# houzhijian/CONE

Measured on AMD Instinct MI355X. Metric: windows/sec + queries/sec, Ego4D-NLQ win_len=90 d=256 top-k=20, higher is better.
Workload: dtype f32

## Files before the change

cone_amd/_lib.py:

```python
from __future__ import annotations

import ctypes as C
import os

HERE = os.path.dirname(os.path.abspath(__file__))
LIB_PATH = os.path.join(HERE, "libcone_hip.so")

MAX_LAYERS = 8
MAX_PROJ = 3

c_float_p = C.c_void_p


class Linear(C.Structure):
    _fields_ = [("w", C.c_void_p), ("b", C.c_void_p)]


class LNorm(C.Structure):
    _fields_ = [("g", C.c_void_p), ("b", C.c_void_p)]


class Mha(C.Structure):
    _fields_ = [("in_proj_w", C.c_void_p), ("in_proj_b", C.c_void_p), ("out_proj", Linear)]

# ... 73 lines not shown
    "cone_topk_windows_workspace": (C.c_size_t, [C.c_int, C.c_int64, C.c_int]),
    "cone_topk_windows_ws": (C.c_int, [C.c_void_p, C.c_int, C.c_int64, C.c_int, C.c_void_p, C.c_void_p, C.c_void_p,
                                       C.c_size_t, C.c_void_p]),
    "cone_project_workspace": (C.c_size_t, [C.c_void_p, C.c_int, C.c_int64]),
    "cone_project_tokens": (C.c_int, [C.c_void_p, C.c_int, C.c_void_p, C.c_int64, C.c_void_p, C.c_void_p,
                                      C.c_size_t, C.c_void_p]),
    "cone_mask_lengths": (C.c_int, [C.c_void_p, C.c_int, C.c_int, C.c_void_p, C.c_void_p]),
    "cone_forward_workspace": (C.c_size_t, [C.c_void_p, C.c_int, C.c_int, C.c_int]),
    "cone_forward_windows": (C.c_int, [C.c_void_p, C.c_void_p, C.c_void_p, C.c_void_p, C.c_void_p, C.c_int,
                                       C.c_int, C.c_int, C.c_void_p, C.c_void_p, C.c_void_p, C.POINTER(Taps),
                                       C.c_void_p, C.c_size_t, C.c_void_p]),
    "cone_forward_packed_workspace": (C.c_size_t, [C.c_void_p, C.c_int, C.c_int, C.c_int, C.POINTER(Layer0)]),
    "cone_forward_packed": (C.c_int, [C.c_void_p, C.c_void_p, C.c_void_p, C.c_void_p, C.c_void_p, C.c_void_p,
                                      C.c_void_p, C.c_int, C.c_int, C.c_int, C.c_void_p, C.c_void_p, C.c_void_p,
                                      C.POINTER(Taps), C.POINTER(Layer0), C.c_void_p, C.c_size_t, C.c_void_p]),
    "cone_pos_table_rows": (C.c_int64, [C.c_int]),
    "cone_pos_tables": (C.c_int, [C.c_void_p, C.c_int, C.c_void_p, C.c_void_p, C.c_void_p]),
    "cone_layer0_project_workspace": (C.c_size_t, [C.c_void_p, C.c_int64]),
    "cone_layer0_project": (C.c_int, [C.c_void_p, C.c_void_p, C.c_int64, C.c_void_p, C.c_void_p, C.c_size_t, C.c_void_p]),
    "cone_layer0_text_positions": (C.c_int, [C.c_void_p, C.c_void_p, C.c_void_p, C.c_int64, C.c_void_p, C.c_void_p, C.c_void_p]),
    "cone_clip_matching_workspace": (C.c_size_t, [C.c_void_p, C.c_int]),
    "cone_clip_matching_gathered": (C.c_int, [C.c_void_p, C.c_void_p, C.c_void_p, C.c_void_p, C.c_void_p,
                                              C.c_void_p, C.c_void_p, C.c_void_p, C.c_int, C.c_void_p,
                                              C.c_void_p, C.c_size_t, C.c_void_p]),
    "cone_clip_matching": (C.c_int, [C.c_void_p, C.c_void_p, C.c_void_p, C.c_void_p, C.c_int, C.c_void_p,
                                     C.c_int, C.c_void_p, C.c_void_p, C.c_size_t, C.c_void_p]),
    "cone_window_table": (C.c_int, [C.c_void_p, C.c_int, C.c_int, C.c_void_p, C.c_void_p, C.c_int] + [C.c_void_p] * 4 + [C.c_int] * 3
                          + [C.c_void_p, C.c_int, C.c_int] + [C.c_void_p] * 7 + [C.c_void_p]),
    "cone_compose_rows": (C.c_int, [C.c_void_p, C.c_void_p, C.c_void_p, C.c_void_p, C.c_void_p, C.c_float,
                                    C.c_int, C.c_int, C.c_int, C.c_void_p, C.c_void_p]),
    "cone_fuse_nms": (C.c_int, [C.c_void_p, C.c_void_p, C.c_void_p, C.c_int, C.c_int, C.c_double, C.c_int, C.c_int,
                                C.c_void_p, C.c_void_p, C.c_void_p, C.c_void_p]),
    "cone_fuse_nms_f64": (C.c_int, [C.c_void_p, C.c_void_p, C.c_void_p, C.c_int, C.c_int, C.c_double, C.c_int, C.c_int,
                                    C.c_void_p, C.c_void_p, C.c_void_p, C.c_void_p]),
    "cone_temporal_nms": (C.c_int, [C.c_void_p, C.c_int, C.c_double, C.c_int, C.c_void_p, C.c_void_p,
                                    C.c_void_p]),
    "cone_matcher_cost": (C.c_int, [C.c_void_p, C.c_void_p, C.c_void_p, C.c_int, C.c_int, C.c_float, C.c_float,
                                    C.c_float, C.c_void_p, C.c_void_p, C.c_void_p]),
    "cone_criterion_forward": (C.c_int, [C.c_void_p, C.c_void_p, C.c_void_p, C.c_void_p, C.c_void_p, C.c_void_p, C.c_int,
                                         C.c_void_p, C.c_void_p, C.c_int, C.c_void_p, C.c_int, C.c_int, C.c_int,
                                         C.c_float, C.c_float, C.c_float, C.c_float, C.c_float, C.c_void_p, C.c_void_p,
                                         C.c_void_p, C.c_void_p]),
    "cone_adapter_nce": (C.c_int, [C.c_void_p, C.c_int, C.c_float, C.c_void_p, C.c_void_p]),
    "cone_prof_enable": (C.c_int, [C.c_int]),
    "cone_prof_collect": (C.c_int64, [C.c_void_p, C.c_int64]),
    "cone_eval_recall": (C.c_int, [C.c_void_p, C.c_void_p, C.c_void_p, C.c_int, C.c_int, C.c_void_p, C.c_int,
                                   C.c_void_p, C.c_int, C.c_int, C.c_void_p, C.c_void_p, C.c_void_p]),
    "cone_eval_window_recall": (C.c_int, [C.c_void_p, C.c_int, C.c_int, C.c_void_p, C.c_double, C.c_int, C.c_void_p,
                                          C.c_int, C.c_void_p, C.c_void_p]),
    "cone_model_set_option": (C.c_int, [C.c_void_p, C.c_char_p, C.c_int]),
    "cone_test_gemm": (C.c_int, [C.c_void_p, C.c_void_p, C.c_int, C.c_void_p, C.c_void_p, C.c_void_p,
                                 C.c_void_p, C.c_void_p, C.c_void_p, C.c_void_p, C.c_void_p, C.c_int, C.c_int,
                                 C.c_int, C.c_int, C.c_void_p]),
    "cone_test_gemm_bf16_image_bytes": (C.c_size_t, [C.c_int, C.c_int]),
    "cone_test_gemm_bf16": (C.c_int, [C.c_void_p, C.c_void_p, C.c_int, C.c_void_p, C.c_void_p, C.c_void_p,
                                      C.c_void_p, C.c_void_p, C.c_void_p, C.c_void_p, C.c_void_p, C.c_int, C.c_int,
                                      C.c_int, C.c_int, C.c_void_p, C.c_int, C.c_int, C.c_void_p, C.c_void_p]),
    "cone_test_ffn": (C.c_int, [C.c_void_p] * 8 + [C.c_int, C.c_int, C.c_void_p]),
    "cone_test_proj_ffn": (C.c_int, [C.c_void_p] * 13 + [C.c_int, C.c_int, C.c_void_p]),
    "cone_test_tail_form": (C.c_int, [C.c_void_p] * 13 + [C.c_int, C.c_int] + [C.c_void_p] * 3 + [C.c_int, C.c_void_p, C.c_int, C.c_int,
                                                                               C.c_void_p, C.c_void_p]),
    "cone_test_proj_ffn_spread_scratch_bytes": (C.c_size_t, [C.c_int]),
    "cone_test_proj_ffn_spread": (C.c_int, [C.c_void_p] * 13 + [C.c_int, C.c_int, C.c_void_p, C.c_void_p]),
    "cone_test_ffn_split_image_bytes": (C.c_size_t, [C.c_int]),
    "cone_test_ffn_split": (C.c_int, [C.c_void_p] * 8 + [C.c_int, C.c_int, C.c_void_p, C.c_int, C.c_void_p]),
    "cone_test_rows_split_image_bytes": (C.c_size_t, [C.c_int]),
    "cone_test_rows_split": (C.c_int, [C.c_void_p] * 4 + [C.c_int, C.c_int, C.c_void_p, C.c_int, C.c_void_p]),
    "cone_test_proj_split_image_bytes": (C.c_size_t, []),
    "cone_test_proj_ffn_split": (C.c_int, [C.c_void_p] * 13 + [C.c_int, C.c_int, C.c_void_p, C.c_void_p, C.c_int, C.c_void_p]),
    "cone_test_enc_attn": (C.c_int, [C.c_int] + [C.c_void_p] * 9 + [C.c_int, C.c_int, C.c_int, C.c_void_p]),
    "cone_test_dec_cross": (C.c_int, [C.c_void_p] * 9 + [C.c_int] * 4 + [C.c_void_p, C.c_void_p]),
    "cone_test_dec_cross_slab_floats": (C.c_size_t, []),
    "cone_test_enc_attn_txt": (C.c_int, [C.c_int] + [C.c_void_p] * 10 + [C.c_int, C.c_int, C.c_int, C.c_void_p]),
    "cone_test_small_attn": (C.c_int, [C.c_void_p, C.c_int, C.c_void_p, C.c_int, C.c_void_p, C.c_int, C.c_void_p, C.c_int,
                                       C.c_void_p, C.c_int, C.c_int, C.c_int, C.c_void_p]),
    "cone_test_dec_cross_ex": (C.c_int, [C.c_void_p] * 10 + [C.c_int] * 4 + [C.c_void_p] * 4 + [C.c_int, C.c_void_p]),
    "cone_test_layernorm": (C.c_int, [C.c_void_p, C.c_void_p, C.c_void_p, C.c_void_p, C.c_int64, C.c_int,
                                      C.c_void_p]),
    "cone_test_gen_attn": (C.c_int, [C.c_void_p, C.c_int, C.c_void_p, C.c_int, C.c_void_p, C.c_int, C.c_void_p, C.c_int,
                                     C.c_void_p, C.c_void_p] + [C.c_int] * 5 + [C.c_void_p]),
    "cone_test_grid_limit_y": (C.c_int, []),
    "cone_test_scan_lengths": (C.c_int, [C.c_void_p, C.c_void_p, C.c_int, C.c_void_p, C.c_void_p]),
    "cone_test_compact_index": (C.c_int, [C.c_void_p, C.c_void_p, C.c_int, C.c_void_p, C.c_void_p, C.c_void_p, C.c_int,
                                          C.c_void_p, C.c_int, C.c_void_p]),
    "cone_test_pack_pos": (C.c_int, [C.c_void_p] * 11 + [C.c_int, C.c_int] + [C.c_void_p] * 4),
    "cone_test_gen_pack_pos": (C.c_int, [C.c_void_p] * 10 + [C.c_int] * 3 + [C.c_void_p] * 4),
    "cone_test_pack_l0": (C.c_int, [C.c_void_p] * 15 + [C.c_int, C.c_int, C.c_void_p]),
    "cone_test_row_index": (C.c_int, [C.c_void_p] * 6 + [C.c_int, C.c_int, C.c_void_p]),
    "cone_test_add_pos_rows": (C.c_int, [C.c_void_p] * 5 + [C.c_int, C.c_int] + [C.c_void_p] * 3),
    "cone_test_txt_pos_rows": (C.c_int, [C.c_void_p] * 3 + [C.c_int, C.c_int] + [C.c_void_p] * 3 + [C.c_int] + [C.c_void_p] * 3),
    "cone_test_gen_txt_pos_rows": (C.c_int, [C.c_void_p] * 3 + [C.c_int, C.c_int] + [C.c_void_p] * 3 + [C.c_int, C.c_void_p, C.c_int,
                                                                                                    C.c_void_p, C.c_void_p]),
    "cone_test_saliency": (C.c_int, [C.c_void_p] * 7 + [C.c_int, C.c_void_p, C.c_int, C.c_int, C.c_void_p]),
    "cone_test_gen_saliency": (C.c_int, [C.c_void_p] * 7 + [C.c_int, C.c_void_p, C.c_int, C.c_int, C.c_int, C.c_void_p]),
    "cone_test_rowdot": (C.c_int, [C.c_void_p, C.c_int, C.c_void_p, C.c_void_p, C.c_void_p, C.c_int, C.c_int64, C.c_int, C.c_int,
                                   C.c_void_p]),
    "cone_test_gen_rowdot": (C.c_int, [C.c_void_p, C.c_int, C.c_void_p, C.c_void_p, C.c_void_p, C.c_int, C.c_int64, C.c_int, C.c_int,
                                       C.c_int, C.c_void_p]),
    "cone_test_tile_rows": (C.c_int, [C.c_void_p, C.c_int, C.c_int64, C.c_void_p]),
    "cone_test_tile_rows2": (C.c_int, [C.c_void_p] * 4 + [C.c_int, C.c_int64, C.c_void_p]),
}
EXPORTS = tuple(_SIGNATURES)

_lib = None


# ... 66 lines not shown
```

cone_amd/build.py:

```python
from __future__ import annotations

import os
import subprocess
import sys
from concurrent.futures import ThreadPoolExecutor

HERE = os.path.dirname(os.path.abspath(__file__))
CSRC = os.path.join(HERE, "csrc")
OBJ = os.path.join(CSRC, "_obj")
LIB = os.path.join(HERE, "libcone_hip.so")
PYLISTS = os.path.join(HERE, "_cone_pylists.so")
SOURCES = ["api.hip", "gemm.hip", "rowops.hip", "attention.hip", "window_ops.hip", "prefilter.hip",
           "postproc.hip", "prof.hip", "dec_cross.hip", "metrics.hip", "ffn.hip", "criterion.hip", "dec_cross_mfma.hip", "ffn_split.hip", "ffn_wide.hip",
           "general.hip", "ffn_bf16.hip", "gemm_bf16.hip"]
FLAGS = ["-O3", "--offload-arch=gfx950", "-fPIC", "-std=c++17", "-Wall", "-Wno-unused-function"]
NO_CONTRACT = {"window_ops.hip", "postproc.hip", "metrics.hip", "criterion.hip", "general.hip"}


def _deps_mtime():
    hdrs = [os.path.join(CSRC, f) for f in os.listdir(CSRC) if f.endswith(".h")]
    hdrs += [os.path.join(HERE, "..", "include", "cone_hip.h"), __file__]
    return max(os.path.getmtime(h) for h in hdrs)


def _compile(src):
    obj = os.path.join(OBJ, src.replace(".hip", ".o"))
    stamp = obj + ".flags"
    path = os.path.join(CSRC, src)
    extra = ["-ffp-contract=off"] if src in NO_CONTRACT else []
    extra += os.environ.get("CONE_HIPCC_FLAGS", "").split()
    flags = " ".join([*FLAGS, *extra])
    try:
        with open(stamp) as f:
            same_flags = f.read() == flags
    except OSError:
        same_flags = False
    if same_flags and os.path.exists(obj) and os.path.getmtime(obj) >= max(os.path.getmtime(path), _deps_mtime()):
        return obj
    cmd = ["hipcc", *FLAGS, *extra, "-c", path, "-o", obj]
    r = subprocess.run(cmd, capture_output=True, text=True)
    if r.returncode != 0:
        raise RuntimeError(f"hipcc failed for {src}:\n{r.stdout}\n{r.stderr}")
    with open(stamp, "w") as f:
        f.write(flags)
    if r.stderr.strip():
        sys.stderr.write(r.stderr)
    return obj


def build(force: bool = False) -> str:
    os.makedirs(OBJ, exist_ok=True)
    if force:
        for f in os.listdir(OBJ):
            os.remove(os.path.join(OBJ, f))
    with ThreadPoolExecutor(max_workers=4) as ex:
        objs = list(ex.map(_compile, SOURCES))
    if (not os.path.exists(LIB)) or any(os.path.getmtime(o) > os.path.getmtime(LIB) for o in objs):
        r = subprocess.run(["hipcc", "--offload-arch=gfx950", "-shared", "-fPIC", "-o", LIB, *objs],
                           capture_output=True, text=True)
        if r.returncode != 0:
            raise RuntimeError(f"link failed:\n{r.stdout}\n{r.stderr}")
    try:
        build_pylists()
    except (RuntimeError, OSError) as e:
        try:
            if os.path.exists(PYLISTS) and os.path.getmtime(PYLISTS) < os.path.getmtime(os.path.join(CSRC, "pylists.c")):
                os.remove(PYLISTS)
# ... 22 lines not shown
```

cone_amd/csrc/api.hip:

```cpp
#include <stdarg.h>
#include <string.h>

#include <vector>

#include "common.h"
#include "rows_chain.h"

namespace cone {

static thread_local char g_err[512] = "";
void set_error(const char* fmt, ...) {
    va_list ap;
    va_start(ap, fmt);
    vsnprintf(g_err, sizeof(g_err), fmt, ap);
    va_end(ap);
}

struct Linear { const float* w = nullptr; const float* b = nullptr; };
struct LNorm { const float* g = nullptr; const float* b = nullptr; };
struct Mha { const float* in_w = nullptr; const float* in_b = nullptr; Linear out; };
struct EncLayer { Mha sa; Linear l1, l2; LNorm n1, n2; };
struct DecLayer { Mha sa, ca; Linear l1, l2; LNorm n1, n2, n3; };

}

struct cone_model {
    int d, heads, ff, n_enc, n_dec, nq, n_proj, dt, dv, dvm, has_adapter;
    float* arena = nullptr;
    cone::LNorm vproj_ln[CONE_MAX_PROJ], tproj_ln[CONE_MAX_PROJ];
    cone::Linear vproj[CONE_MAX_PROJ], tproj[CONE_MAX_PROJ];
    cone::EncLayer enc[CONE_MAX_LAYERS];
    cone::DecLayer dec[CONE_MAX_LAYERS];
    cone::LNorm dec_norm;
    const float* query_embed = nullptr;
    cone::Linear class_embed, span[3], saliency, adapter[2];
    const float* dim_t = nullptr;
    const float* txt_pos_emb = nullptr; int txt_pos_rows = 0; cone::LNorm txt_pos_ln;
    int pre_norm = 0; cone::LNorm enc_norm;
    cone::Linear dec_k, dec_v;
    const float* dec_vT[CONE_MAX_LAYERS] = {};
    float* dec0_tgt1 = nullptr; float* dec0_dq = nullptr; float* dec0_scratch = nullptr;
    float* dec_sa_tab[CONE_MAX_LAYERS] = {}; float* dec_ca_tab[CONE_MAX_LAYERS] = {};
    float* tab_arena = nullptr; const float* tab_pos_rows = nullptr; const float* tab_pos_qk = nullptr; int tab_max_v_l = 0;
    int opt_dec_fold = 2;
    int opt_dec0_const = 1;
    int opt_l0_gather = 1;
    int opt_pos_tables = 1;
    int opt_gemm = 0;
    cone::TailWeights enc_tail[CONE_MAX_LAYERS] = {}, dec_tail[CONE_MAX_LAYERS] = {};
    char* split_img = nullptr; char* bf16_img = nullptr;
    int opt_qkv_fused = 1;
    int opt_split_bf16 = 0;
    int opt_bf16 = 0;
    int opt_res_gather = 1;
    int opt_spread = 1;
    int opt_chain = 1;
    int opt_ffn_fused = 2;
    int gen_native = 0;
// ... 1528 lines not shown
                                      void* stream) {
    return launch_gen_pack_pos(vproj, vrow0, vlen, tproj, trow0, qlen, off, dim_t, X, POS, d, B, Lmax, (hipStream_t)stream, tpe,
                               tpg, tpb);
}
extern "C" int cone_test_pack_l0(const float* vproj, const int32_t* vrow0, const int32_t* vlen, const float* tproj,
                                 const int32_t* trow0, const int32_t* qlen, const int32_t* off, const float* dim_t,
                                 const float* qkv_vid, const float* qkv_txt, const float* pos_qk, float* X, float* POS, float* QK,
                                 float* V, int B, int Lmax, void* stream) {
    return launch_pack_l0(vproj, vrow0, vlen, tproj, trow0, qlen, off, dim_t, qkv_vid, qkv_txt, pos_qk, X, POS, QK, V, B, Lmax,
                          (hipStream_t)stream);
}
extern "C" int cone_test_row_index(const int32_t* vrow0, const int32_t* vlen, const int32_t* trow0, const int32_t* qlen,
                                   const int32_t* off, int32_t* ridx, int B, int Lmax, void* stream) {
    return launch_row_index(vrow0, vlen, trow0, qlen, off, ridx, B, Lmax, (hipStream_t)stream);
}
extern "C" int cone_test_add_pos_rows(const float* MEM, const int32_t* off, const int32_t* vlen, const float* pos_rows, float* XP,
                                      int B, int Lmax, const float* txt_pos, const int32_t* trow0, void* stream) {
    return launch_add_pos_rows(MEM, off, vlen, pos_rows, XP, B, Lmax, (hipStream_t)stream, txt_pos, trow0);
}
extern "C" int cone_test_txt_pos_rows(const float* tproj, const int32_t* tok_index, const int32_t* src_row, int mod, int n_emb,
                                      const float* tpe, const float* tpg, const float* tpb, int n, const int32_t* n_dev,
                                      float* out, void* stream) {
    return launch_txt_pos_rows(tproj, tok_index, src_row, mod, n_emb, tpe, tpg, tpb, n, n_dev, out, (hipStream_t)stream);
}
extern "C" int cone_test_gen_txt_pos_rows(const float* tproj, const int32_t* tok_index, const int32_t* src_row, int mod, int n_emb,
                                          const float* tpe, const float* tpg, const float* tpb, int n, const int32_t* n_dev, int d,
                                          float* out, void* stream) {
    return launch_gen_txt_pos_rows(tproj, tok_index, src_row, mod, n_emb, tpe, tpg, tpb, n, n_dev, d, out, (hipStream_t)stream);
}
extern "C" int cone_test_saliency(const float* MEM, const int32_t* off, const int32_t* vlen, const int32_t* qlen, const float* w,
                                  const float* bias, float* sal, int Lv_out, float* mem_tap, int Lq_out, int B, void* stream) {
    return launch_saliency(MEM, off, vlen, qlen, w, bias, sal, Lv_out, mem_tap, Lq_out, B, (hipStream_t)stream);
}
extern "C" int cone_test_gen_saliency(const float* MEM, const int32_t* off, const int32_t* vlen, const int32_t* qlen,
                                      const float* w, const float* bias, float* sal, int Lv_out, float* mem_tap, int Lq_out, int B,
                                      int d, void* stream) {
    return launch_gen_saliency(MEM, off, vlen, qlen, w, bias, sal, Lv_out, mem_tap, Lq_out, B, d, (hipStream_t)stream);
}
extern "C" int cone_test_rowdot(const float* X, int ldx, const float* W, const float* b, float* out, int ldo, int64_t n_rows,
                                int nout, int act, void* stream) {
    return launch_rowdot(X, ldx, W, b, out, ldo, n_rows, nout, act, (hipStream_t)stream);
}
extern "C" int cone_test_gen_rowdot(const float* X, int ldx, const float* W, const float* b, float* out, int ldo, int64_t n_rows,
                                    int nout, int act, int d, void* stream) {
    return launch_gen_rowdot(X, ldx, W, b, out, ldo, n_rows, nout, act, d, (hipStream_t)stream);
}
extern "C" int cone_test_tile_rows(float* x, int period, int64_t n_rows, void* stream) {
    return launch_tile_rows(x, period, n_rows, (hipStream_t)stream);
}
extern "C" int cone_test_tile_rows2(float* d0, const float* s0, float* d1, const float* s1, int period, int64_t n_rows,
                                    void* stream) {
    return launch_tile_rows2(d0, s0, d1, s1, period, n_rows, (hipStream_t)stream);
}
```

cone_amd/csrc/gemm.hip:

```cpp
#include <mutex>

#include "common.h"
#include "rows_chain.h"

#ifndef CONE_GEMM_NT_STORE
#define CONE_GEMM_NT_STORE 0
#endif

namespace cone {

constexpr int BK = 32;

template <int BM, int BN, bool HAS_A2>
__global__ __launch_bounds__(256, 2) void gemm_f32_kernel(GemmArgs p) {
    constexpr int WAVES_N = BN / 64;
    constexpr int LDA_S = BM + 1, LDB_S = BN + 1;
    constexpr int A_PASSES = BM / 32, B_PASSES = BN / 32;
    __shared__ float smem[BK * LDA_S + BK * LDB_S];
    float* As = smem;
    float* Bs = smem + BK * LDA_S;

    int M = p.M;
    if (p.M_dev) { int md = *p.M_dev; M = md < M ? md : M; }
    const int m0 = blockIdx.x * BM;
    if (m0 >= M) return;
    const int n0 = blockIdx.y * BN;
    const int N = p.N, K = p.K;

    const int tid = threadIdx.x;
    const int lane = tid & 63;
    const int wave = tid >> 6;
    const int wm = wave / WAVES_N, wn = wave % WAVES_N;
    const int li = lane & 31, lh = lane >> 5;

    const int lrow = tid >> 3;
    const int lkc = tid & 7;

    float4 ra[A_PASSES], rb[B_PASSES];

    auto gload = [&](int kt) {
        const int kof = kt * BK + lkc * 4;
#pragma unroll
        for (int ps = 0; ps < A_PASSES; ++ps) {
            int row = m0 + lrow + 32 * ps;
            row = row < M ? row : M - 1;
            float4 v = *reinterpret_cast<const float4*>(p.A + (size_t)row * p.lda + kof);
            if (HAS_A2) {
                const int r2 = p.a2_mod ? row % p.a2_mod : row;
                const float4 w = *reinterpret_cast<const float4*>(p.A2 + (size_t)r2 * p.lda2 + kof);
                v.x += w.x; v.y += w.y; v.z += w.z; v.w += w.w;
            }
            ra[ps] = v;
        }
#pragma unroll
        for (int ps = 0; ps < B_PASSES; ++ps) {
// ... 293 lines not shown
#pragma unroll
    for (int g = 0; g < 4; ++g) {
        __builtin_amdgcn_wave_barrier();
#pragma unroll
        for (int t = 0; t < 8; ++t)
#pragma unroll
            for (int rr4 = 0; rr4 < 4; ++rr4)
                ep[(rr4 + 4 * lh) * RT_EP_LD + t * 32 + li] = acc[t][4 * g + rr4];
        __builtin_amdgcn_wave_barrier();
        float4 v[8], rr[8], ad[8];
#pragma unroll
        for (int k = 0; k < 8; ++k) {
            int i = min(8 * g + k, rows_here - 1);
            i = i < 0 ? 0 : i;
            const size_t m = (size_t)min(mrow0 + i, M - 1);
            if (flags & EPI_RESIDUAL) rr[k] = *reinterpret_cast<const float4*>(p.R + (p.r_mod ? m % (size_t)p.r_mod : m) * p.ldr + n0 + c4);
            if (p.C2) ad[k] = *reinterpret_cast<const float4*>(p.ADD + m * p.ldc + n0 + c4);
            v[k] = *reinterpret_cast<const float4*>(ep + k * RT_EP_LD + c4);
        }
#pragma unroll
        for (int k = 0; k < 8; ++k) {
            float4 x = v[k];
            x.x += bias4.x; x.y += bias4.y; x.z += bias4.z; x.w += bias4.w;
            if (flags & EPI_RELU) { x.x = fmaxf(x.x, 0.f); x.y = fmaxf(x.y, 0.f); x.z = fmaxf(x.z, 0.f); x.w = fmaxf(x.w, 0.f); }
            if (flags & EPI_RESIDUAL) { x.x += rr[k].x; x.y += rr[k].y; x.z += rr[k].z; x.w += rr[k].w; }
            if (flags & EPI_LN) {
                const float mean = wave_sum_dpp((x.x + x.y) + (x.z + x.w)) * (1.0f / 256.0f);
                const float d0 = x.x - mean, d1 = x.y - mean, d2 = x.z - mean, d3 = x.w - mean;
                const float var = wave_sum_dpp((d0 * d0 + d1 * d1) + (d2 * d2 + d3 * d3)) * (1.0f / 256.0f);
                const float rstd = 1.0f / sqrtf(var + 1e-5f);
                x.x = d0 * rstd * g4.x + be4.x; x.y = d1 * rstd * g4.y + be4.y;
                x.z = d2 * rstd * g4.z + be4.z; x.w = d3 * rstd * g4.w + be4.w;
            }
            if (8 * g + k < rows_here) {
                const size_t m = (size_t)(mrow0 + 8 * g + k);
                *reinterpret_cast<float4*>(p.C + m * p.ldc + n0 + c4) = x;
                if (p.C2) {
                    x.x += ad[k].x; x.y += ad[k].y; x.z += ad[k].z; x.w += ad[k].w;
                    *reinterpret_cast<float4*>(p.C2 + m * p.ldc + n0 + c4) = x;
                }
            }
        }
    }
}

typedef float f32x4a __attribute__((ext_vector_type(4)));

__device__ __forceinline__ int swz16(int row) { return (0x1230 >> (((row >> 2) & 3) * 4)) & 3; }

__global__ __launch_bounds__(512, 4) void gemm_rows16_kernel(GemmArgs p) {
    constexpr int RBK = 16, SLAB = (RT_BM + RT_BN) * RBK, NBUF = 3, NPIECE = 3;
    extern __shared__ __attribute__((aligned(16))) float smem[];
    int M = p.M;
    if (p.M_dev) { int md = *p.M_dev; M = md < M ? md : M; }
    const int nc = p.N / RT_BN;
    const int L = blockIdx.x, grp = L / (8 * nc), r0 = L % (8 * nc);
    const int m0 = (grp * 8 + (r0 & 7)) * RT_BM;
    if (m0 >= M) return;
    const int n0 = (r0 >> 3) * RT_BN;
    const int K = p.K;
    const int tid = threadIdx.x, lane = tid & 63;
    const int wave = __builtin_amdgcn_readfirstlane(tid >> 6);
    const int li = lane & 15, lg = lane >> 4;

    const float* __restrict__ Ab = p.A + (size_t)m0 * p.lda;
    const float* __restrict__ Wb = p.W + (size_t)n0 * p.ldw;
    const float* src[NPIECE];
    int dst[NPIECE];
#pragma unroll
    for (int i = 0; i < NPIECE; ++i) {
        const int q = wave * NPIECE + i;
        const int row = q * 16 + lane / 4;
        const int chunk = (lane % 4) ^ swz16(row);
        if (q < 8) {
            const int sr = (m0 + row < M) ? row : (M - 1 - m0);
            src[i] = Ab + (size_t)sr * p.lda + (chunk << 2);
        } else {
            src[i] = Wb + (size_t)(row - RT_BM) * p.ldw + (chunk << 2);
        }
        dst[i] = q * 256;
    }
    auto stream_piece = [&](int kt, int buf, int i) { GLDS16(src[i] + kt * RBK, smem + buf * SLAB + dst[i]); };

    f32x4a acc[16];
#pragma unroll
    for (int t = 0; t < 16; ++t) acc[t] = f32x4a{0.f, 0.f, 0.f, 0.f};
    const int csw = (lg ^ swz16(li)) << 2;
    const int a_row = (wave * 16 + li) * RBK + csw;
    const int b_row = RT_BM * RBK + li * RBK + csw;

    const int nk = K / RBK;
#pragma unroll
    for (int i = 0; i < NPIECE; ++i) stream_piece(0, 0, i);
    if (nk > 1) {
#pragma unroll
        for (int i = 0; i < NPIECE; ++i) stream_piece(1, 1, i);
        asm volatile("s_waitcnt vmcnt(%0)" ::"n"(NPIECE) : "memory");
    } else {
        asm volatile("s_waitcnt vmcnt(0)" ::: "memory");
    }
    __builtin_amdgcn_s_barrier();
    for (int kt = 0; kt < nk; ++kt) {
        const float* sb = smem + (kt % NBUF) * SLAB;
        const int nxt = (kt + 2) % NBUF;
        const bool more = kt + 2 < nk;
        const f32x4a a = *reinterpret_cast<const f32x4a*>(sb + a_row);
#pragma unroll
// ... 375 lines not shown
#pragma unroll
            for (int t = 0; t < 2; ++t)
#pragma unroll
                for (int r = 0; r < 4; ++r) ep[(4 * lg + r) * RS_EP_LD + 32 * wave + 16 * t + li] = acc[t][r];
            __syncthreads();
            const int flags = st.flags;
            float4 bias4 = make_float4(0.f, 0.f, 0.f, 0.f);
            if (st.bias) bias4 = *reinterpret_cast<const float4*>(st.bias + c4);
            float4 v[2], rr[2];
#pragma unroll
            for (int k = 0; k < 2; ++k) {
                const size_t m = (size_t)min(m0 + 2 * wave + k, M - 1);
                if (flags & EPI_RESIDUAL) rr[k] = *reinterpret_cast<const float4*>(st.R + m * st.ldr + c4);
                v[k] = *reinterpret_cast<const float4*>(ep + (2 * wave + k) * RS_EP_LD + c4);
            }
#pragma unroll
            for (int k = 0; k < 2; ++k) {
                float4 xx = v[k];
                xx.x += bias4.x; xx.y += bias4.y; xx.z += bias4.z; xx.w += bias4.w;
                if (flags & EPI_RELU) { xx.x = fmaxf(xx.x, 0.f); xx.y = fmaxf(xx.y, 0.f); xx.z = fmaxf(xx.z, 0.f); xx.w = fmaxf(xx.w, 0.f); }
                if (flags & EPI_RESIDUAL) { xx.x += rr[k].x; xx.y += rr[k].y; xx.z += rr[k].z; xx.w += rr[k].w; }
                x[k] = xx;
            }
        }
        in_regs = true;
#pragma unroll
        for (int k = 0; k < 2; ++k) {
            const int m = m0 + 2 * wave + k;
            if (st.C && m < M) *reinterpret_cast<float4*>(st.C + (size_t)m * st.ldc + c4) = x[k];
            if (st.hout) {
                for (int n = 0; n < st.hnout; ++n) {
                    const float4 xv = x[k];
                    const float4 wv = reinterpret_cast<const float4*>(st.hw + n * 256)[lane];
                    float s = __builtin_fmaf(xv.x, wv.x, xv.y * wv.y) + __builtin_fmaf(xv.z, wv.z, xv.w * wv.w);
                    s = wave_sum(s) + st.hb[n];
                    if (st.hact == 1) s = 1.0f / (1.0f + expf(-s));
                    if (lane == 0 && m < M) st.hout[(size_t)m * st.hld + n] = s;
                }
            }
        }
    }
    asm volatile("s_waitcnt vmcnt(0)" ::: "memory");
}


#ifndef CONE_RS_MAX_WGS
#define CONE_RS_MAX_WGS 1280
#endif
constexpr int RS_MAX_WGS = CONE_RS_MAX_WGS;
#ifndef CONE_RS_SPLIT_WGS
#define CONE_RS_SPLIT_WGS 256
#endif

int launch_gemm(const GemmArgs& a, hipStream_t s) {
    CONE_REQUIRE(a.K > 0 && a.K % BK == 0, "gemm: K=%d must be a multiple of %d", a.K, BK);
    CONE_REQUIRE(a.lda % 4 == 0 && a.ldw % 4 == 0, "gemm: lda/ldw must be multiples of 4");
    CONE_REQUIRE(!(a.flags & EPI_RESIDUAL) || a.R, "gemm: residual flag without R");
    if (a.M <= 0) return 0;
    if (a.flags & EPI_LN) CONE_REQUIRE(a.N == 256 && a.ln_g && a.ln_b, "gemm: LayerNorm epilogue needs N == 256");
    const bool rows_ok = a.N % 256 == 0 && !a.A2;
    const bool use_rows = rows_ok && a.variant != GEMM_SQUARE;
    const bool need_rows = a.C2 != nullptr;
    CONE_REQUIRE(!need_rows || (rows_ok && a.ADD), "gemm: second output needs the row tile (N %% 256 == 0, no A2)");
    if (use_rows || need_rows) {
        static DeviceOnce once;
        CONE_CHECK_HIP(device_once(once, [] {
            hipError_t rc = hipFuncSetAttribute((const void*)gemm_rows16_kernel, hipFuncAttributeMaxDynamicSharedMemorySize,
                                                RowTile<16>::LDS_BYTES);
            if (rc == hipSuccess)
                rc = hipFuncSetAttribute((const void*)gemm_rows_kernel<16>, hipFuncAttributeMaxDynamicSharedMemorySize,
                                         RowTile<16>::LDS_BYTES);
            if (rc == hipSuccess)
                rc = hipFuncSetAttribute((const void*)gemm_rows_small_kernel, hipFuncAttributeMaxDynamicSharedMemorySize, 160 * 1024);
            return rc;
        }));
        int n_cu = 0;
        CONE_CHECK_HIP(device_once(once, [] { return hipSuccess; }, &n_cu));
        const bool waves8 = a.variant != GEMM_ROWS4;
        const bool small_ok = waves8 && !a.C2 && a.variant == GEMM_AUTO && rs_lds_bytes(a.K) <= 160 * 1024;
        if (small_ok && (int64_t)((a.M + 15) / 16) * (a.N / RT_BN) > RS_MAX_WGS && a.m_off == 0) {
            const int nc = a.N / RT_BN;
            const int64_t G = (int64_t)((a.M + RT_BM - 1) / RT_BM) * nc;
            const int64_t m1 = G / n_cu * n_cu / nc * RT_BM;
            const int64_t rem = a.M - m1;
            if (m1 > 0 && rem > 0 && (rem + 15) / 16 * nc <= CONE_RS_SPLIT_WGS) {
                GemmArgs h = a;
                h.M = (int)m1;
                h.variant = GEMM_ROWS8;
                if (int rc = launch_gemm(h, s)) return rc;
                GemmArgs t = a;
                t.A = a.A + (size_t)m1 * a.lda; t.C = a.C + (size_t)m1 * a.ldc; t.M = (int)rem; t.m_off = (int)m1;
                if (a.R && !a.r_mod) t.R = a.R + (size_t)m1 * a.ldr;
                return launch_gemm(t, s);
            }
        }
        if (small_ok && !(a.flags & EPI_LN) && a.K <= 1024 && (a.M + 15) / 16 <= RSP_MAX_GROUPS &&
            (a.M + 15) / 16 * (a.N / 16) <= RSP_MAX_TILES && !(a.flags & GEMM_NO_SPREAD)) {
            ProfScope ps(PK_GEMM_ROWS_SMALL, a.M, a.N, a.K, a.M_dev, s, a.m_off);
            hipLaunchKernelGGL(gemm_rows_spread_kernel, dim3((unsigned)(a.N / 16), (unsigned)((a.M + 15) / 16)), dim3(64), 0, s, a);
            CONE_LAUNCH_CHECK();
            return 0;
        }
        if (small_ok && (int64_t)((a.M + 15) / 16) * (a.N / RT_BN) <= RS_MAX_WGS) {
            ProfScope ps(PK_GEMM_ROWS_SMALL, a.M, a.N, a.K, a.M_dev, s, a.m_off);
            hipLaunchKernelGGL(gemm_rows_small_kernel, dim3((unsigned)((a.M + 15) / 16), (unsigned)(a.N / RT_BN)), dim3(512),
                               rs_lds_bytes(a.K), s, a);
            CONE_LAUNCH_CHECK();
            return 0;
        }
        const int row_tiles = (a.M + RT_BM - 1) / RT_BM;
        dim3 grid((unsigned)((row_tiles + 7) / 8 * 8 * (a.N / RT_BN)));
        ProfScope ps(waves8 ? PK_GEMM_ROWS16 : PK_GEMM_ROWS, a.M, a.N, a.K, a.M_dev, s);
        if (waves8)
            hipLaunchKernelGGL(gemm_rows16_kernel, grid, dim3(512), RowTile<16>::LDS_BYTES, s, a);
        else
            hipLaunchKernelGGL(gemm_rows_kernel<16>, grid, dim3(256), RowTile<16>::LDS_BYTES, s, a);
        CONE_LAUNCH_CHECK();
        return 0;
    }
    if (a.flags & EPI_LN) {
        CONE_REQUIRE(a.N == 256 && a.ln_g && a.ln_b, "gemm: LayerNorm epilogue needs N == 256");
        CONE_REQUIRE(!a.A2, "gemm: LayerNorm epilogue with A2 is not instantiated");
        dim3 grid((a.M + 63) / 64, 1);
        ProfScope ps(PK_GEMM_64x256, a.M, a.N, a.K, a.M_dev, s);
        hipLaunchKernelGGL((gemm_f32_kernel<64, 256, false>), grid, dim3(256), 0, s, a);
    } else {
        dim3 grid((a.M + 127) / 128, (a.N + 127) / 128);
        ProfScope ps(a.A2 ? PK_GEMM_128x128_A2 : PK_GEMM_128x128, a.M, a.N, a.K, a.M_dev, s);
        if (a.A2) {
            CONE_REQUIRE(a.lda2 % 4 == 0, "gemm: lda2 must be a multiple of 4");
            hipLaunchKernelGGL((gemm_f32_kernel<128, 128, true>), grid, dim3(256), 0, s, a);
        } else {
            hipLaunchKernelGGL((gemm_f32_kernel<128, 128, false>), grid, dim3(256), 0, s, a);
        }
    }
    CONE_LAUNCH_CHECK();
    return 0;
}

bool rows_chain_supported(int M) { return M > 0 && (M + 15) / 16 <= RS_MAX_WGS; }
bool gemm_rows_spread_rows(int M) { return M > 0 && (M + 15) / 16 <= RSP_MAX_GROUPS; }

int launch_rows_chain(const ChainArgs& a, hipStream_t s) {
    CONE_REQUIRE(a.A && a.n_stages >= 1 && a.n_stages <= CHAIN_MAX_STAGES && a.lda % 4 == 0, "rows chain: bad arguments");
    if (a.M <= 0) return 0;
    CONE_REQUIRE(rows_chain_supported(a.M), "rows chain: %d rows are beyond the small-M regime", a.M);
    for (int i = 0; i < a.n_stages; ++i) {
        const ChainStage& st = a.st[i];
        if (st.kind == 0) {
            CONE_REQUIRE(st.W && st.K % 16 == 0 && st.K >= 16 && st.K <= 1024 && (i == 0 || st.K == 256),
                         "rows chain: stage %d: K=%d (stage 0: a multiple of 16 up to 1024; later stages: 256)", i, st.K);
            CONE_REQUIRE(!(st.flags & EPI_RESIDUAL) || (st.R && st.ldr % 4 == 0), "rows chain: residual flag without R");
            CONE_REQUIRE(!(st.flags & EPI_LN), "rows chain: a LayerNorm epilogue is a stage of its own (kind 1)");
        } else {
            CONE_REQUIRE(st.kind == 1 && st.ln_g && st.ln_b, "rows chain: stage %d: bad LayerNorm stage", i);
        }
        CONE_REQUIRE(!st.C || st.ldc % 4 == 0, "rows chain: output row stride must be a multiple of 4");
        CONE_REQUIRE(!st.hout || (st.hw && st.hb && st.hnout >= 1 && st.hnout <= 2), "rows chain: bad head");
    }
    CONE_REQUIRE(a.st[0].kind == 0 || a.lda >= 256, "rows chain: a LayerNorm first stage reads 256-wide rows");
    const int K0 = a.st[0].kind == 0 ? a.st[0].K : 256;
    const size_t lds = (size_t)((16 * K0 > 16 * RS_EP_LD ? 16 * K0 : 16 * RS_EP_LD) + 16 * RS_EP_LD + 8 * RS_RING) * sizeof(float);
    static DeviceOnce once;
    CONE_CHECK_HIP(device_once(once, [] {
        return hipFuncSetAttribute((const void*)rows_chain_kernel, hipFuncAttributeMaxDynamicSharedMemorySize, 160 * 1024);
    }));
    hipLaunchKernelGGL(rows_chain_kernel, dim3((unsigned)((a.M + 15) / 16)), dim3(512), lds, s, a);
    CONE_LAUNCH_CHECK();
    return 0;
}

}
```

include/cone_hip.h:

```cpp
#ifndef CONE_HIP_H
#define CONE_HIP_H

#include <stddef.h>
#include <stdint.h>

#ifdef __cplusplus
extern "C" {
#endif

#define CONE_HIP_ABI_VERSION 8

#define CONE_E_INVALID (-1)
#define CONE_E_HIP (-2)
#define CONE_E_WORKSPACE (-3)

#define CONE_MAX_LAYERS 8
#define CONE_MAX_PROJ 3
#define CONE_TABLE_MAX_V_L 255
#define CONE_MAX_WINDOW_TOKENS 256
#define CONE_MAX_LONG_WINDOW_TOKENS 1024

typedef struct cone_model cone_model;

typedef struct { const float* w; const float* b; } cone_linear_w;
// ... 133 lines not shown
                        const int32_t* txt_len, int B, int Lv_max, int Lq_max,
                        float* logits, float* spans, float* saliency, const cone_taps* taps,
                        const cone_layer0* l0 , void* ws, size_t ws_bytes, void* stream);

size_t cone_clip_matching_workspace(const cone_model* m, int B);
int cone_clip_matching_gathered(const cone_model* m, const float* cls, const int32_t* cls_row,
                                const float* vid, const int32_t* vid_row0, const int32_t* vid_len,
                                const int32_t* pad_len, const float* spans, int B, float* match,
                                void* ws, size_t ws_bytes, void* stream);
int cone_clip_matching(const cone_model* m, const float* cls, const float* vid, const int32_t* vid_len,
                       int Lv_pad, const float* spans, int B, float* match,
                       void* ws, size_t ws_bytes, void* stream);

int cone_compose_rows(const float* logits, const float* spans, const float* match,
                      const int32_t* duration, const int32_t* video_start, float clip_length,
                      int sort, int B, int Nq, float* rows, void* stream);


int cone_fuse_nms(const float* cand, const int64_t* cand_off, const int32_t* n_valid, int nq, int n_max,
                  double nms_thd, int max_before, int max_after, double* out_rows, int32_t* out_n, int32_t* out_idx,
                  void* stream);

int cone_fuse_nms_f64(const double* cand, const int64_t* cand_off, const int32_t* n_valid, int nq, int n_max,
                      double nms_thd, int max_before, int max_after, double* out_rows, int32_t* out_n, int32_t* out_idx,
                      void* stream);

int cone_temporal_nms(const double* pred, int n, double nms_thd, int max_after,
                      int32_t* keep_idx, int32_t* keep_n, void* stream);

int cone_matcher_cost(const float* logits, const float* spans, const float* tgt, int B, int Nq,
                      float cost_span, float cost_giou, float cost_class, float* cost, int32_t* best,
                      void* stream);

int cone_criterion_forward(const float* logits, const float* spans, const float* tgt, const int32_t* tgt_off,
                           const float* neg_logits, const float* saliency, int L, const int32_t* pos_idx,
                           const int32_t* neg_idx, int P, const float* neg_saliency, int L2, int B, int Nq,
                           float cost_span, float cost_giou, float cost_class, float eos_coef, float saliency_margin,
                           int32_t* assign, float* part, float* losses, void* stream);
int cone_adapter_nce(const float* sim, int n, float temperature, float* loss, void* stream);

int cone_eval_recall(const double* rows, const int32_t* n, const double* gt, int nq, int max_after,
                     const double* thresholds, int n_thr, const int32_t* topk, int n_topk, int mode,
                     int64_t* hits, double* top1_iou, void* stream);
int cone_eval_window_recall(const int32_t* win_idx, int nq, int k, const double* gt, double clip_length,
                            int slide, const int32_t* topk, int n_topk, int64_t* hits, void* stream);

int cone_prof_enable(int on);
int64_t cone_prof_collect(double* out, int64_t max_rec);

int cone_model_set_option(cone_model* m, const char* name, int value);
int cone_test_gemm(const float* A, const float* A2, int a2_mod, const float* W, const float* bias,
                   const float* R, const float* ln_g, const float* ln_b, float* C, float* C2,
                   const float* ADD, int M, int N, int K, int flags, void* stream);
size_t cone_test_gemm_bf16_image_bytes(int N, int K);
int cone_test_gemm_bf16(const float* A, const float* A2, int a2_mod, const float* W, const float* bias,
                        const float* R, const float* ln_g, const float* ln_b, float* C, float* C2,
                        const float* ADD, int M, int N, int K, int flags, void* img, int ldc, int r_mod,
                        const int32_t* M_dev, void* stream);
int cone_test_ffn(const float* X, const float* W1, const float* b1, const float* W2, const float* b2,
                  const float* ln_g, const float* ln_b, float* OUT, int M, int ff, void* stream);
int cone_test_proj_ffn(const float* A, const float* Wo, const float* bo, const float* R, const float* pg, const float* pb,
                       const float* W1, const float* b1, const float* W2, const float* b2, const float* ln_g,
                       const float* ln_b, float* OUT, int M, int ff, void* stream);
#define CONE_TEST_PACK 1
#define CONE_TEST_SINGLE_PIECE 2
size_t cone_test_ffn_split_image_bytes(int ff);
int cone_test_ffn_split(const float* X, const float* W1, const float* b1, const float* W2, const float* b2,
                        const float* ln_g, const float* ln_b, float* OUT, int M, int ff, void* img, int pack, void* stream);
size_t cone_test_rows_split_image_bytes(int N);
int cone_test_rows_split(const float* X, const float* W, const float* bias, float* C, int M, int N, void* img, int pack,
                         void* stream);
#define CONE_FFN_SPREAD_MAX_ROWS 1024
size_t cone_test_proj_ffn_spread_scratch_bytes(int ff);
int cone_test_proj_ffn_spread(const float* A, const float* Wo, const float* bo, const float* R, const float* pg, const float* pb,
                              const float* W1, const float* b1, const float* W2, const float* b2, const float* ln_g,
                              const float* ln_b, float* OUT, int M, int ff, void* scratch, void* stream);
enum { CONE_TAIL_FORM_ROWS128 = 0, CONE_TAIL_FORM_ROWS64 = 1, CONE_TAIL_FORM_WIDE = 2, CONE_TAIL_FORM_LADDER = 3,
       CONE_TAIL_FORM_SPREAD = 4 };
int cone_test_tail_form(const float* A, const float* Wo, const float* bo, const float* R, const float* pg, const float* pb,
                        const float* W1, const float* b1, const float* W2, const float* b2, const float* ln_g,
                        const float* ln_b, float* OUT, int M, int ff, const int32_t* r_idx, const float* R2,
                        const int32_t* M_dev, int pre, float* OUT2, int form, int n_cu, void* scratch, void* stream);
size_t cone_test_proj_split_image_bytes(void);
int cone_test_proj_ffn_split(const float* A, const float* Wo, const float* bo, const float* R, const float* pg,
                             const float* pb, const float* W1, const float* b1, const float* W2, const float* b2,
                             const float* ln_g, const float* ln_b, float* OUT, int M, int ff, void* img, void* wo_img,
                             int pack, void* stream);
int cone_test_enc_attn(int mode, const float* QKV, const float* qkv_vid, const float* qkv_txt, const float* pos_qk,
                       const int32_t* vrow0, const int32_t* vlen, const int32_t* trow0, const int32_t* off, float* OUT,
                       int B, int Lmax, int pos_zero_row , void* stream);
int cone_test_dec_cross(const float* DQ, const float* X, const float* pos_rows, const int32_t* vlen, const int32_t* off,
                        const float* Wk, const float* WvT, const float* bv, float* OUT, int B, int nq, int Lmax,
                        int variant, float* qk_slabs, void* stream);
size_t cone_test_dec_cross_slab_floats(void);
int cone_test_enc_attn_txt(int mode, const float* QKV, const float* qkv_vid, const float* qkv_txt, const float* pos_qk,
                           const float* txt_pos_qk, const int32_t* vrow0, const int32_t* vlen, const int32_t* trow0,
                           const int32_t* off, float* OUT, int B, int Lmax, int pos_zero_row, void* stream);
int cone_test_small_attn(const float* Q, int ldq, const float* K, int ldk, const float* V, int ldv, float* OUT, int ldo,
                         const int32_t* off, int B, int nq, int Lmax, void* stream);
int cone_test_dec_cross_ex(const float* DQ, const float* XP, const float* X, const float* pos_rows, const int32_t* vlen,
                           const int32_t* off, const float* Wk, const float* WvT, const float* bv, float* OUT, int B, int nq,
                           int Lmax, int variant, float* qk_slabs, const float* sal_w, const float* sal_b, float* sal,
                           int sal_ld, void* stream);
int cone_test_layernorm(const float* x, const float* g, const float* b, float* out, int64_t n_rows,
                        int dim, void* stream);
int cone_test_gen_attn(const float* Q, int ldq, const float* K, int ldk, const float* V, int ldv, float* OUT, int ldo,
// ... 41 lines not shown
```

Measured before the change: 376,200.

## Add persistent MFMA GEMM for K=256 bias-only projections with tail fallback

Result: no change. 379,100, median of 6 (+0.8%).

```diff
diff --git a/cone_amd/_lib.py b/cone_amd/_lib.py
--- a/cone_amd/_lib.py
+++ b/cone_amd/_lib.py
@@ -149,6 +149,9 @@
     "cone_test_gemm": (C.c_int, [C.c_void_p, C.c_void_p, C.c_int, C.c_void_p, C.c_void_p, C.c_void_p,
                                  C.c_void_p, C.c_void_p, C.c_void_p, C.c_void_p, C.c_void_p, C.c_int, C.c_int,
                                  C.c_int, C.c_int, C.c_void_p]),
+    "cone_test_gemm_ladder": (C.c_int, [C.c_void_p, C.c_void_p, C.c_int, C.c_void_p, C.c_void_p, C.c_void_p,
+                                        C.c_void_p, C.c_void_p, C.c_void_p, C.c_void_p, C.c_void_p, C.c_int, C.c_int,
+                                        C.c_int, C.c_int, C.c_int, C.c_void_p, C.c_int, C.c_void_p]),
     "cone_test_gemm_bf16_image_bytes": (C.c_size_t, [C.c_int, C.c_int]),
     "cone_test_gemm_bf16": (C.c_int, [C.c_void_p, C.c_void_p, C.c_int, C.c_void_p, C.c_void_p, C.c_void_p,
                                       C.c_void_p, C.c_void_p, C.c_void_p, C.c_void_p, C.c_void_p, C.c_int, C.c_int,
diff --git a/cone_amd/build.py b/cone_amd/build.py
--- a/cone_amd/build.py
+++ b/cone_amd/build.py
@@ -12,7 +12,7 @@
 PYLISTS = os.path.join(HERE, "_cone_pylists.so")
 SOURCES = ["api.hip", "gemm.hip", "rowops.hip", "attention.hip", "window_ops.hip", "prefilter.hip",
            "postproc.hip", "prof.hip", "dec_cross.hip", "metrics.hip", "ffn.hip", "criterion.hip", "dec_cross_mfma.hip", "ffn_split.hip", "ffn_wide.hip",
-           "general.hip", "ffn_bf16.hip", "gemm_bf16.hip"]
+           "general.hip", "ffn_bf16.hip", "gemm_bf16.hip", "gemm_persist.hip"]
 FLAGS = ["-O3", "--offload-arch=gfx950", "-fPIC", "-std=c++17", "-Wall", "-Wno-unused-function"]
 NO_CONTRACT = {"window_ops.hip", "postproc.hip", "metrics.hip", "criterion.hip", "general.hip"}
 
diff --git a/cone_amd/csrc/api.hip b/cone_amd/csrc/api.hip
--- a/cone_amd/csrc/api.hip
+++ b/cone_amd/csrc/api.hip
@@ -4,6 +4,7 @@
 #include <vector>
 
 #include "common.h"
+#include "gemm_persist.h"
 #include "rows_chain.h"
 
 namespace cone {
@@ -1638,3 +1639,13 @@
                                     void* stream) {
     return launch_tile_rows2(d0, s0, d1, s1, period, n_rows, (hipStream_t)stream);
 }
+extern "C" int cone_test_gemm_ladder(const float* A, const float* A2, int a2_mod, const float* W, const float* bias,
+                                     const float* R, const float* ln_g, const float* ln_b, float* C, float* C2,
+                                     const float* ADD, int M, int N, int K, int flags, int ldc, const int32_t* M_dev, int n_cu,
+                                     void* stream) {
+    GemmArgs g = G(nullptr, A, K, W, K, bias, C, ldc ? ldc : N, M, M_dev, N, K, flags & 0xff);
+    g.variant = (flags >> 8) & 3;
+    g.A2 = A2; g.lda2 = K; g.a2_mod = a2_mod; g.R = R; g.ldr = N; g.ln_g = ln_g; g.ln_b = ln_b;
+    g.C2 = C2; g.ADD = ADD;
+    return launch_gemm_ladder(g, n_cu, (hipStream_t)stream);
+}
diff --git a/cone_amd/csrc/gemm.hip b/cone_amd/csrc/gemm.hip
--- a/cone_amd/csrc/gemm.hip
+++ b/cone_amd/csrc/gemm.hip
@@ -1,6 +1,7 @@
 #include <mutex>
 
 #include "common.h"
+#include "gemm_persist.h"
 #include "rows_chain.h"
 
 #ifndef CONE_GEMM_NT_STORE
@@ -400,7 +401,7 @@
     constexpr int RBK = 16, SLAB = (RT_BM + RT_BN) * RBK, NBUF = 3, NPIECE = 3;
     extern __shared__ __attribute__((aligned(16))) float smem[];
     int M = p.M;
-    if (p.M_dev) { int md = *p.M_dev; M = md < M ? md : M; }
+    if (p.M_dev) { int md = *p.M_dev - p.m_off; M = md < M ? md : M; }
     const int nc = p.N / RT_BN;
     const int L = blockIdx.x, grp = L / (8 * nc), r0 = L % (8 * nc);
     const int m0 = (grp * 8 + (r0 & 7)) * RT_BM;
@@ -882,7 +883,7 @@
 #define CONE_RS_SPLIT_WGS 256
 #endif
 
-int launch_gemm(const GemmArgs& a, hipStream_t s) {
+static int launch_gemm_on(const GemmArgs& a, hipStream_t s, int n_cu_as) {
     CONE_REQUIRE(a.K > 0 && a.K % BK == 0, "gemm: K=%d must be a multiple of %d", a.K, BK);
     CONE_REQUIRE(a.lda % 4 == 0 && a.ldw % 4 == 0, "gemm: lda/ldw must be multiples of 4");
     CONE_REQUIRE(!(a.flags & EPI_RESIDUAL) || a.R, "gemm: residual flag without R");
@@ -906,6 +907,22 @@
         }));
         int n_cu = 0;
         CONE_CHECK_HIP(device_once(once, [] { return hipSuccess; }, &n_cu));
+        if (n_cu_as > 0) n_cu = n_cu_as;
+#if CONE_GEMM_PERSIST
+        if (a.variant == GEMM_AUTO && gemm_persist_supported(a) && a.ldc % 4 == 0) {
+            const int64_t round = (int64_t)GP_ROWS * n_cu;
+            const int64_t m1 = a.M / round * round;
+            if (m1 > 0) {
+                GemmArgs h = a;
+                h.M = (int)m1;
+                if (int rc = launch_gemm_persist(h, n_cu, s)) return rc;
+                if (m1 == a.M) return 0;
+                GemmArgs t = a;
+                t.A = a.A + (size_t)m1 * a.lda; t.C = a.C + (size_t)m1 * a.ldc; t.M = (int)(a.M - m1); t.m_off = (int)m1;
+                return launch_gemm_on(t, s, n_cu_as);
+            }
+        }
+#endif
         const bool waves8 = a.variant != GEMM_ROWS4;
         const bool small_ok = waves8 && !a.C2 && a.variant == GEMM_AUTO && rs_lds_bytes(a.K) <= 160 * 1024;
         if (small_ok && (int64_t)((a.M + 15) / 16) * (a.N / RT_BN) > RS_MAX_WGS && a.m_off == 0) {
@@ -917,11 +934,11 @@
                 GemmArgs h = a;
                 h.M = (int)m1;
                 h.variant = GEMM_ROWS8;
-                if (int rc = launch_gemm(h, s)) return rc;
+                if (int rc = launch_gemm_on(h, s, n_cu_as)) return rc;
                 GemmArgs t = a;
                 t.A = a.A + (size_t)m1 * a.lda; t.C = a.C + (size_t)m1 * a.ldc; t.M = (int)rem; t.m_off = (int)m1;
                 if (a.R && !a.r_mod) t.R = a.R + (size_t)m1 * a.ldr;
-                return launch_gemm(t, s);
+                return launch_gemm_on(t, s, n_cu_as);
             }
         }
         if (small_ok && !(a.flags & EPI_LN) && a.K <= 1024 && (a.M + 15) / 16 <= RSP_MAX_GROUPS &&
@@ -940,7 +957,7 @@
         }
         const int row_tiles = (a.M + RT_BM - 1) / RT_BM;
         dim3 grid((unsigned)((row_tiles + 7) / 8 * 8 * (a.N / RT_BN)));
-        ProfScope ps(waves8 ? PK_GEMM_ROWS16 : PK_GEMM_ROWS, a.M, a.N, a.K, a.M_dev, s);
+        ProfScope ps(waves8 ? PK_GEMM_ROWS16 : PK_GEMM_ROWS, a.M, a.N, a.K, a.M_dev, s, waves8 ? a.m_off : 0);
         if (waves8)
             hipLaunchKernelGGL(gemm_rows16_kernel, grid, dim3(512), RowTile<16>::LDS_BYTES, s, a);
         else
@@ -968,6 +985,12 @@
     return 0;
 }
 
+int launch_gemm(const GemmArgs& a, hipStream_t s) { return launch_gemm_on(a, s, 0); }
+int launch_gemm_ladder(const GemmArgs& a, int n_cu, hipStream_t s) {
+    CONE_REQUIRE(n_cu > 0, "gemm ladder hook: needs a CU count");
+    return launch_gemm_on(a, s, n_cu);
+}
+
 bool rows_chain_supported(int M) { return M > 0 && (M + 15) / 16 <= RS_MAX_WGS; }
 bool gemm_rows_spread_rows(int M) { return M > 0 && (M + 15) / 16 <= RSP_MAX_GROUPS; }
 
diff --git a/cone_amd/csrc/gemm_persist.h b/cone_amd/csrc/gemm_persist.h
--- /dev/null
+++ b/cone_amd/csrc/gemm_persist.h
@@ -0,0 +1,17 @@
+#pragma once
+
+#include "common.h"
+
+namespace cone {
+
+#ifndef CONE_GEMM_PERSIST
+#define CONE_GEMM_PERSIST 1
+#endif
+
+constexpr int GP_ROWS = 128;
+
+bool gemm_persist_supported(const GemmArgs& a);
+int launch_gemm_persist(const GemmArgs& a, int grid, hipStream_t s);
+int launch_gemm_ladder(const GemmArgs& a, int n_cu, hipStream_t s);
+
+}
diff --git a/cone_amd/csrc/gemm_persist.hip b/cone_amd/csrc/gemm_persist.hip
--- /dev/null
+++ b/cone_amd/csrc/gemm_persist.hip
@@ -0,0 +1,165 @@
+#include "gemm_persist.h"
+#include "tail_f32_common.h"
+
+namespace cone {
+
+constexpr int GP_NW = 8;
+constexpr int GP_K = 256;
+constexpr int GP_STAGE = 32 * GP_K;
+constexpr int GP_NST = 4;
+constexpr int GP_NPIECE = 32 / GP_NW;
+constexpr int GP_MAX_N = 4096;
+static_assert(GP_ROWS == 16 * GP_NW, "a wave owns 16 rows of the tile");
+static_assert(GP_NPIECE == 4, "the chunk's units 0 .. 3 issue one piece each; the chunk's counted wait leaves exactly these "
+                              "GP_NPIECE youngest entries of the vmcnt queue outstanding");
+constexpr int GP_SYNC_UNIT = 6;
+static_assert(GP_SYNC_UNIT >= GP_NPIECE - 1 && GP_SYNC_UNIT < 7, "the chunk's pieces are issued ahead of its wait; unit 7 prefetches behind it");
+static_assert((GP_NST & (GP_NST - 1)) == 0 && GP_NST >= 4, "stage index is masked; chunk c + 2 must not land in a stage still read");
+
+static size_t gp_lds_bytes(int N) { return (size_t)(GP_NST * GP_STAGE + N) * sizeof(float); }
+
+#define GP_SB() __builtin_amdgcn_sched_barrier(0)
+#define GP_RD(stg, off) (*reinterpret_cast<const f32x4*>((stg) + (off) + rd))
+#define GP_MFMA(acc, a, b) { acc = __builtin_amdgcn_mfma_f32_16x16x4f32(a, b, acc, 0, 0, 0); GP_SB(); }
+
+#define GP_LANDED(v) asm volatile("" : "+v"(v));
+#define GP_CHUNK(LAST)                                                                                                     \
+    {                                                                                                                      \
+        const float* st = smem + cs * GP_STAGE;                                                                            \
+        const float* sn = smem + ((cs + 1) & (GP_NST - 1)) * GP_STAGE;                                                     \
+        const int ns = (cs + 2) & (GP_NST - 1);                                                                            \
+        f32x4 ha = f32x4{0.f, 0.f, 0.f, 0.f}, hb = ha;                                                                     \
+        if (LAST) {                                                                                                        \
+            _Pragma("unroll") for (int q = 0; q < 16; ++q) xn[q] = *reinterpret_cast<const f32x4*>(xnp + 16 * q);          \
+        }                                                                                                                  \
+        _Pragma("unroll") for (int u = 0; u < 8; ++u) {                                                                    \
+            GP_SB();                                                                                                       \
+            asm volatile("" : "+v"(wa), "+v"(wb), "+v"(va), "+v"(vb));                                                     \
+            GP_SB();                                                                                                       \
+            if (u < 7) {                                                                                                   \
+                na = GP_RD(st, (2 * u + 2) * 256); nb = GP_RD(st, (2 * u + 3) * 256);                                      \
+                nva = GP_RD(st, 4096 + (2 * u + 2) * 256); nvb = GP_RD(st, 4096 + (2 * u + 3) * 256);                      \
+            } else {                                \
+                na = GP_RD(sn, 0); nb = GP_RD(sn, 256); nva = GP_RD(sn, 4096); nvb = GP_RD(sn, 4096 + 256);                \
+            }                                                                                                              \
+            GP_SB();                                                                                                       \
+            _Pragma("unroll") for (int r = 0; r < 4; ++r) {                                                                \
+                GP_MFMA(ha, wa[r], x[2 * u][r])                                                                            \
+                GP_MFMA(hb, va[r], x[2 * u][r])                                                                            \
+            }                                                                                                              \
+            _Pragma("unroll") for (int r = 0; r < 4; ++r) {                                                                \
+                GP_MFMA(ha, wb[r], x[2 * u + 1][r])                                                                        \
+                GP_MFMA(hb, vb[r], x[2 * u + 1][r])                                                                        \
+            }                                                                                                              \
+            if (u < GP_NPIECE) stream_piece(gs, ns, u);                                                                    \
+            if (u == GP_SYNC_UNIT) {                                                                                       \
+                GP_SB();                                                                                                   \
+                asm volatile("s_waitcnt vmcnt(%0)" ::"n"(GP_NPIECE) : "memory");                                           \
+                __builtin_amdgcn_s_barrier();                                                                              \
+                GP_SB();                                                                                                   \
+            }                                                                                                              \
+            wa = na; wb = nb; va = nva; vb = nvb;                                                                          \
+        }                                                                                                                  \
+        GP_SB();                                                                                                           \
+        const f32x4 o0 = ha + *reinterpret_cast<const f32x4*>(bs + 32 * g + 4 * lg);                                       \
+        const f32x4 o1 = hb + *reinterpret_cast<const f32x4*>(bs + 32 * g + 16 + 4 * lg);                                  \
+        GP_SB();                                                                                                           \
+        if (LAST) {                                                                                                        \
+            _Pragma("unroll") for (int q = 0; q < 16; ++q) { x[q] = xn[q]; GP_LANDED(x[q]) }                               \
+            GP_SB();                                                                                                       \
+        }                                                                                                                  \
+        if (row_ok) {                                                                                                      \
+            *reinterpret_cast<f32x4*>(crow + 32 * g) = o0;                                                                 \
+            *reinterpret_cast<f32x4*>(crow + 32 * g + 16) = o1;                                                            \
+        }                                                                                                                  \
+        GP_SB();                                                                                                           \
+        cs = (cs + 1) & (GP_NST - 1);                                                                                      \
+        gs = gs + 1 == G ? 0 : gs + 1;                                                                                     \
+    }
+
+__global__ __launch_bounds__(64 * GP_NW, 2) void gemm_rows_persist_kernel(GemmArgs p) {
+    extern __shared__ __attribute__((aligned(16))) float smem[];
+    float* bs = smem + GP_NST * GP_STAGE;
+    TF_LAUNCH_ROWS(M, p, 0)
+    const int n_tiles = (M + GP_ROWS - 1) / GP_ROWS;
+    if ((int)blockIdx.x >= n_tiles) return;
+    const int tid = threadIdx.x, lane = tid & 63;
+    const int wave = __builtin_amdgcn_readfirstlane(tid >> 6);
+    const int li = lane & 15, lg = lane >> 4;
+    const int N = p.N, G = N >> 5;
+
+    for (int i = tid; i < (N >> 2); i += 64 * GP_NW)
+        reinterpret_cast<f32x4*>(bs)[i] = p.bias ? reinterpret_cast<const f32x4*>(p.bias)[i] : f32x4{0.f, 0.f, 0.f, 0.f};
+
+    const int drow = lane >> 2;
+    const int dch = (lane & 3) ^ tf_swz16(drow);
+    const unsigned vo = (unsigned)(((16 * (wave >> 2) + drow) * p.ldw + 16 * GP_NPIECE * (wave & 3) + 4 * dch) * 4);
+    auto stream_piece = [&](int gg, int stage, int i) {
+        float* dstp = smem + stage * GP_STAGE + (wave * GP_NPIECE + i) * 256;
+        const char* ub = reinterpret_cast<const char*>(p.W + ((size_t)gg * 32 * p.ldw + 16 * i));
+        asm volatile("" : "+s"(ub));
+        TF_GLDS16(ub + vo, dstp);
+    };
+    const int rd = li * 16 + ((lg ^ tf_swz16(li)) << 2);
+
+    f32x4 x[16], xn[16];
+    auto row_ptr = [&](int tile) { return p.A + TF_LD_ROW(tile * GP_ROWS + wave * 16 + li, M) * p.lda + 4 * lg; };
+    {
+        const float* xp = row_ptr(blockIdx.x);
+#pragma unroll
+        for (int q = 0; q < 16; ++q) x[q] = *reinterpret_cast<const f32x4*>(xp + 16 * q);
+    }
+#pragma unroll
+    for (int i = 0; i < GP_NPIECE; ++i) stream_piece(0, 0, i);
+#pragma unroll
+    for (int i = 0; i < GP_NPIECE; ++i) stream_piece(1 < G ? 1 : 0, 1, i);
+    int cs = 0;
+    int gs = 2 % G;
+    asm volatile("s_waitcnt vmcnt(%0)" ::"n"(GP_NPIECE) : "memory");
+    __syncthreads();
+#pragma unroll
+    for (int q = 0; q < 16; ++q) GP_LANDED(x[q])
+
+    f32x4 wa, wb, na, nb;
+    f32x4 va, vb, nva, nvb;
+    wa = GP_RD(smem, 0); wb = GP_RD(smem, 256); va = GP_RD(smem, 4096); vb = GP_RD(smem, 4096 + 256);
+    for (int tile = blockIdx.x; tile < n_tiles; tile += gridDim.x) {
+        const int my_row = tile * GP_ROWS + wave * 16 + li;
+        const bool row_ok = my_row < M;
+        float* crow = p.C + (size_t)(row_ok ? my_row : 0) * p.ldc + 4 * lg;
+        const float* xnp = row_ptr(tile + (int)gridDim.x < n_tiles ? tile + (int)gridDim.x : tile);
+        int g = 0;
+        for (; g < G - 1; ++g) GP_CHUNK(false)
+        GP_CHUNK(true)
+    }
+    asm volatile("s_waitcnt vmcnt(0)" ::: "memory");
+}
+
+#undef GP_CHUNK
+#undef GP_LANDED
+#undef GP_MFMA
+#undef GP_RD
+#undef GP_SB
+
+bool gemm_persist_supported(const GemmArgs& a) {
+    return a.K == GP_K && a.N >= 32 && a.N % 32 == 0 && a.N <= GP_MAX_N && a.flags == 0 && !a.A2 && !a.C2 && !a.R && a.m_off == 0;
+}
+
+int launch_gemm_persist(const GemmArgs& a, int grid, hipStream_t s) {
+    CONE_REQUIRE(gemm_persist_supported(a), "gemm: the persistent form takes K = 256, N %% 32 == 0, a bias-only epilogue");
+    CONE_REQUIRE(a.lda % 4 == 0 && a.ldw % 4 == 0 && a.ldc % 4 == 0 && grid > 0, "gemm: the persistent form needs 16-B rows");
+    if (a.M <= 0) return 0;
+    static DeviceOnce once;
+    CONE_CHECK_HIP(device_once(once, [] {
+        return hipFuncSetAttribute((const void*)gemm_rows_persist_kernel, hipFuncAttributeMaxDynamicSharedMemorySize,
+                                   (int)gp_lds_bytes(GP_MAX_N));
+    }));
+    const int n_tiles = (a.M + GP_ROWS - 1) / GP_ROWS;
+    ProfScope ps(PK_GEMM_ROWS16, a.M, a.N, a.K, a.M_dev, s);
+    hipLaunchKernelGGL(gemm_rows_persist_kernel, dim3((unsigned)(n_tiles < grid ? n_tiles : grid)), dim3(64 * GP_NW),
+                       gp_lds_bytes(a.N), s, a);
+    CONE_LAUNCH_CHECK();
+    return 0;
+}
+
+}
diff --git a/include/cone_hip.h b/include/cone_hip.h
--- a/include/cone_hip.h
+++ b/include/cone_hip.h
@@ -209,6 +209,10 @@
 int cone_test_gemm(const float* A, const float* A2, int a2_mod, const float* W, const float* bias,
                    const float* R, const float* ln_g, const float* ln_b, float* C, float* C2,
                    const float* ADD, int M, int N, int K, int flags, void* stream);
+int cone_test_gemm_ladder(const float* A, const float* A2, int a2_mod, const float* W, const float* bias,
+                          const float* R, const float* ln_g, const float* ln_b, float* C, float* C2,
+                          const float* ADD, int M, int N, int K, int flags, int ldc, const int32_t* M_dev, int n_cu,
+                          void* stream);
 size_t cone_test_gemm_bf16_image_bytes(int N, int K);
 int cone_test_gemm_bf16(const float* A, const float* A2, int a2_mod, const float* W, const float* bias,
                         const float* R, const float* ln_g, const float* ln_b, float* C, float* C2,
```
